# uzh-rpg/rpg_svo

Hardware: AMD Instinct MI355X
Metric: frames/sec sparse-align+pose-refine (VGA, 4 pyr lvls); ATE vs CPU ref (higher is better)
Workload: dtype value = default build: K1 f32 pixels/residuals/chi2/per-pixel products, f64 Jacobian rows/partials/reductions/projection/solve/pose; K4 f64 (reference-width build: roofline_f64_build.value)

## Files before the change

rpg_svo_amd/csrc/sparse_align.hip:

```cpp
#include <cstdlib>
#include <map>
#include <mutex>
#include <utility>

#include "sia_common.h"

using namespace svo_capi;
using namespace svo_dev;
using namespace svo_sia;

namespace {

#define MINW(BLOCK) ((BLOCK) >= 256 ? 4 : 3)

#ifdef SIA_PROFILE
#define SIA_T() ((long long)__builtin_readcyclecounter())
#define SIA_ACC(k, t0, t1) prof[k] += (t1) - (t0)
#else
#define SIA_T() 0ll
#define SIA_ACC(k, t0, t1)
#endif

constexpr int MAX_WAVES = SVO_HIP_MAX_PATCHES / 64;

#if defined(SIA_F64_PARTIALS)
using sia_pix = double;
using sia_acc = double;
#undef MINW
#define MINW(BLOCK) 3
#else
using sia_pix = float;
using sia_acc = double;
#endif

struct SplitModel {
  double q[2][4], t[2][3];
};

struct SiaLds {
  SplitModel sm;
  double Rt[12];
  int sw_done, sw_stop, sw_nmeas, sw_cur, sw_old;
  double sw_chi2;
  double H[21];
  double Hinv[36];
  double A[36];
  sia_acc part[2][MAX_WAVES][8];
  int chg[2][MAX_WAVES];
  int xfail;
  sia_acc Hpart[MAX_WAVES][24];
  long long lo[SVO_HIP_MAX_LEVELS];
  int lw[SVO_HIP_MAX_LEVELS];
  int lh[SVO_HIP_MAX_LEVELS];
  int lp[SVO_HIP_MAX_LEVELS];
};
__shared__ SiaLds g_s;


template <int PARTS>
__device__ __forceinline__ void sia_rebuild_hinv(int lane, int nw, [[maybe_unused]] XChunk* xh, [[maybe_unused]] int part,
                                                 [[maybe_unused]] unsigned gen, [[maybe_unused]] int& xfail) {
  asm volatile("" : "+v"(lane));
#ifndef SVO_HOST_MATH_TEST
  if constexpr (PARTS > 1) {
    static_assert((PARTS - 1) * 21 <= 64, "one lane per chunk of the other parts");
    const int j = lane / 21, k = lane - 21 * j;
    double v = 0.0;
    for (int w = 0; w < nw; ++w) v += (double)g_s.Hpart[w][k];
    if (j == 0) sia_xstore(xh + part * SIA_XH_SLOTS + k, v, gen);
    const int other = j < part ? j : j + 1;
    double got = 0.0;
    if (j < PARTS - 1) got = sia_xpoll(xh + other * SIA_XH_SLOTS + k, gen, xfail);
    if (xfail) g_s.xfail = 1;
    double tot = 0.0;
#pragma unroll
    for (int p = 0; p < PARTS; ++p) {
      const double theirs = __shfl(got, (p < part ? p : p - 1) * 21 + k, 64);
      const double term = p == part ? v : theirs;
      tot = p == 0 ? term : tot + term;
    }
    if (lane < 21) g_s.H[lane] = tot;
  } else
#endif
  if (lane < 21) {
    double v = 0.0;
    for (int w = 0; w < nw; ++w) v += (double)g_s.Hpart[w][lane];
    g_s.H[lane] = v;
  }
  SVO_WAVE_LDS_FENCE();
  const int gi = lane / 6, gj = lane - 6 * gi;
  if (lane < 36) {
    g_s.A[lane] = g_s.H[sym6_rt(gi, gj)];
    g_s.Hinv[lane] = (gi == gj) ? 1.0 : 0.0;
  }
  for (int k = 0; k < 6; ++k) {
    SVO_WAVE_LDS_FENCE();
    if (lane < 36) {
      const double p = g_s.A[k * 6 + k];
      const double aik = g_s.A[gi * 6 + k];
      const double akj = g_s.A[k * 6 + gj];
      const double bkj = g_s.Hinv[k * 6 + gj];
      const double aij = g_s.A[lane];
      const double bij = g_s.Hinv[lane];
      const double ip = (fabs(p) > 2.2250738585072014e-308) ? sia_rcp(p) : 0.0;
      const double na = (gi == k) ? akj * ip : aij - aik * (akj * ip);
      const double nb = (gi == k) ? bkj * ip : bij - aik * (bkj * ip);
      SVO_LANES_LDS_FENCE();
      g_s.A[lane] = na;
      g_s.Hinv[lane] = nb;
    }
  }
}


__device__ __forceinline__ float sia_bilerp(float wtl, float wtr, float wbl, float wbr, float tl, float tr, float bl, float br) {
  return __builtin_fmaf(wbr, br, __builtin_fmaf(wbl, bl, __builtin_fmaf(wtr, tr, wtl * tl)));
}
typedef float sia_f2 __attribute__((ext_vector_type(2)));
__device__ __forceinline__ sia_f2 sia_bilerp2(sia_f2 wtl, sia_f2 wtr, sia_f2 wbl, sia_f2 wbr, sia_f2 tl, sia_f2 tr, sia_f2 bl,
                                              sia_f2 br) {
  return __builtin_elementwise_fma(wbr, br, __builtin_elementwise_fma(wbl, bl, __builtin_elementwise_fma(wtr, tr, wtl * tl)));
}

#ifdef SIA_F64_PARTIALS
#define SIA_PACKED 0
#else
#define SIA_PACKED 1
#endif
template <int BLOCK, bool WC, bool DIST, int PARTS = 1>
__global__ void __launch_bounds__(BLOCK, PARTS > 1 ? 1 : ((DIST && BLOCK < 1024) ? 3 : MINW(BLOCK))) sia_kernel(const SiaArgs a) {
  constexpr int NW = BLOCK / 64;
  int b, part = 0;
  if constexpr (PARTS > 1) {
    b = (int)(blockIdx.x / (8 * PARTS)) * 8 + (int)(blockIdx.x % 8);
    part = (int)(blockIdx.x / 8) % PARTS;
    if (b >= a.B) return;
  } else {
    b = (int)xcd_contiguous_block();
  }
  [[maybe_unused]] XChunk* const xbase = PARTS > 1 ? static_cast<XChunk*>(a.xw) + (size_t)b * SIA_X_BLOCK : nullptr;
  [[maybe_unused]] unsigned xseq = 0;
#ifndef SVO_HOST_MATH_TEST
  if constexpr (PARTS > 1) xseq = (unsigned)__builtin_amdgcn_readfirstlane((int)sia_xload(xbase + SIA_X_CHUNKS).lo);
#endif
  [[maybe_unused]] int xfail = 0;
  const int tid = threadIdx.x;
  const int lane = tid & 63;
  const int wave = tid >> 6;

  __shared__ float4 s_bt[8][BLOCK];

  int n = a.n[b];
  n = n > a.n_stride ? a.n_stride : n;
  const svo_hip_sia_params P = a.P;

  if (n <= 0) {
    if (tid == 0 && part == 0) {
      for (int k = 0; k < 12; ++k) a.T_out[12 * b + k] = a.T_in[12 * b + k];
      if (a.H_out)
        for (int k = 0; k < 36; ++k) a.H_out[36 * b + k] = 0.0;
      a.n_tracked[b] = 0;
      if (a.iters)
        for (int k = 0; k < SVO_HIP_MAX_LEVELS; ++k) a.iters[SVO_HIP_MAX_LEVELS * b + k] = 0;
      if (a.chi2) a.chi2[b] = 1e10;
      if (a.status) a.status[b] = 0;
    }
    return;
  }

  const int pid = part * BLOCK + tid;
  const size_t fo = (size_t)b * a.n_stride + pid;
  const bool has = (pid < n) && (a.valid ? a.valid[fo] != 0 : true);
  double X = 0, Y = 0, Z = 1;
  if (has) {
    X = a.xyz[3 * fo];
    Y = a.xyz[3 * fo + 1];
    Z = a.xyz[3 * fo + 2];
  }
  double px_kept0 = 0, px_kept1 = 0;
  if (has) {
    px_kept0 = a.px[2 * fo];
    px_kept1 = a.px[2 * fo + 1];
  }
  const double rz = sia_rcp(Z);
  const sia_acc zi = (sia_acc)rz;
  const sia_acc xn = (sia_acc)(X * rz);
  const sia_acc yn = (sia_acc)(Y * rz);
  const uint8_t* ref_base = a.store + (int64_t)a.ref_slot[b] * a.L.slot_bytes;
  const uint8_t* cur_base = a.store + (int64_t)a.cur_slot[b] * a.L.slot_bytes;

  if (tid == 0) {
#pragma unroll
    for (int k = 0; k < SVO_HIP_MAX_LEVELS; ++k) {
      g_s.lw[k] = a.L.w[k];
      g_s.lh[k] = a.L.h[k];
      g_s.lp[k] = a.L.pitch[k];
      g_s.lo[k] = a.L.offset[k];
    }
    for (int k = 0; k < 21; ++k) g_s.H[k] = 0.0;
    g_s.xfail = 0;
    if (a.iters && part == 0)
      for (int k = 0; k < SVO_HIP_MAX_LEVELS; ++k) a.iters[SVO_HIP_MAX_LEVELS * b + k] = 0;
  }
  double R[9], tr[3];
  {
    double q[4];
    for (int k = 0; k < 9; ++k) R[k] = a.T_in[12 * b + k];
    for (int k = 0; k < 3; ++k) tr[k] = a.T_in[12 * b + 9 + k];
    quat_from_R(R, q);
    quat_to_R(q, R);
    if (tid == 0) {
      for (int k = 0; k < 4; ++k) g_s.sm.q[0][k] = q[k];
      for (int k = 0; k < 3; ++k) g_s.sm.t[0][k] = tr[k];
    }
  }
  int m_cur = 0, m_old = 0;
  double chi2_prev = 1e10;
  int stop = 0;
  int n_meas_last = 0;
  int buf = 0;

  const int sw = (NW > 1) ? (int)(blockIdx.x % NW) : 0;
  sia_pix Sxx = 0, Sxy = 0, Syy = 0;
  sia_acc gmask = 0;
  bool vis = false;

  __syncthreads();

#ifdef SIA_PROFILE
  long long prof[8] = {0, 0, 0, 0, 0, 0, 0, 0};
  const long long t_begin = SIA_T();
#endif
  for (int level = P.max_level; level >= P.min_level; --level) {
    [[maybe_unused]] const long long tl0 = SIA_T();
    const int cols = g_s.lw[level], rows = g_s.lh[level], pitch = g_s.lp[level];
    const uint8_t* ref_img = ref_base + g_s.lo[level];
    const uint8_t* cur_img = cur_base + g_s.lo[level];
    const float scale = pow2_inv_f32(level);
    const sia_acc fl = (sia_acc)(fabs(P.fx) * pow2_inv_f64(level));

    uint32_t wc[WC ? 7 : 1][3];
    int wc_u0 = 0, wc_v0 = -100000;
    if (WC) {
#pragma unroll
      for (int r = 0; r < (WC ? 7 : 1); ++r) wc[r][0] = wc[r][1] = wc[r][2] = 0u;
    }
    {
      const double pxx = px_kept0, pxy = px_kept1;
      const float u_ref = (float)(pxx * (double)scale);
      const float v_ref = (float)(pxy * (double)scale);
      const int u_i = (int)floorf(u_ref);
      const int v_i = (int)floorf(v_ref);
      const bool inb = has && !(u_i - 3 < 0 || v_i - 3 < 0 || u_i + 3 >= cols || v_i + 3 >= rows);
      Sxx = Sxy = Syy = 0;
      if (inb) {
        vis = true;
        gmask = 1;
        const float su = u_ref - (float)u_i, sv = v_ref - (float)v_i;
        const float wtl = (1.f - su) * (1.f - sv);
        const float wtr = su * (1.f - sv);
        const float wbl = (1.f - su) * sv;
        const float wbr = su * sv;
        float Bt[6][6];
        float Wp[7], Wc[7];
        uint32_t rw[7][3];
        const int rxa = run_start(u_i - 3, 7);
        const uint32_t rbo = (uint32_t)(u_i - 3 - rxa);
        load_window12<7>(ref_img, pitch, rxa, v_i - 3, rw);
        cut_row7(rw[0], rbo, Wp);
#pragma unroll
        for (int r = 0; r < 6; ++r) {
          cut_row7(rw[r + 1], rbo, Wc);
#pragma unroll
          for (int c = 0; c < 6; ++c) {
            const bool need = ((r >= 1 && r <= 4)) || ((c >= 1 && c <= 4));
            if (need) Bt[r][c] = sia_bilerp(wtl, wtr, wbl, wbr, Wp[c], Wp[c + 1], Wc[c], Wc[c + 1]);
          }
#pragma unroll
          for (int c = 0; c < 7; ++c) Wp[c] = Wc[c];
        }
#pragma unroll
        for (int y = 0; y < 4; ++y)
#pragma unroll
          for (int x = 0; x < 4; ++x) {
            const float dx = 0.5f * (Bt[y + 1][x + 2] - Bt[y + 1][x]);
            const float dy = 0.5f * (Bt[y + 2][x + 1] - Bt[y][x + 1]);
            Sxx += (sia_pix)dx * (sia_pix)dx;
            Sxy += (sia_pix)dx * (sia_pix)dy;
            Syy += (sia_pix)dy * (sia_pix)dy;
          }
#if SIA_PACKED
        s_bt[0][tid] = make_float4(Bt[0][1], Bt[0][3], Bt[0][2], Bt[0][4]);
        s_bt[1][tid] = make_float4(Bt[1][0], Bt[1][2], Bt[1][1], Bt[1][3]);
        s_bt[2][tid] = make_float4(Bt[1][4], Bt[1][5], Bt[2][0], Bt[2][2]);
        s_bt[3][tid] = make_float4(Bt[2][1], Bt[2][3], Bt[2][4], Bt[2][5]);
        s_bt[4][tid] = make_float4(Bt[3][0], Bt[3][2], Bt[3][1], Bt[3][3]);
        s_bt[5][tid] = make_float4(Bt[3][4], Bt[3][5], Bt[4][0], Bt[4][2]);
        s_bt[6][tid] = make_float4(Bt[4][1], Bt[4][3], Bt[4][4], Bt[4][5]);
        s_bt[7][tid] = make_float4(Bt[5][1], Bt[5][3], Bt[5][2], Bt[5][4]);
#else
        s_bt[0][tid] = make_float4(Bt[0][1], Bt[0][2], Bt[0][3], Bt[0][4]);
        s_bt[1][tid] = make_float4(Bt[1][0], Bt[1][1], Bt[1][2], Bt[1][3]);
        s_bt[2][tid] = make_float4(Bt[1][4], Bt[1][5], Bt[2][0], Bt[2][1]);
        s_bt[3][tid] = make_float4(Bt[2][2], Bt[2][3], Bt[2][4], Bt[2][5]);
        s_bt[4][tid] = make_float4(Bt[3][0], Bt[3][1], Bt[3][2], Bt[3][3]);
        s_bt[5][tid] = make_float4(Bt[3][4], Bt[3][5], Bt[4][0], Bt[4][1]);
        s_bt[6][tid] = make_float4(Bt[4][2], Bt[4][3], Bt[4][4], Bt[4][5]);
        s_bt[7][tid] = make_float4(Bt[5][1], Bt[5][2], Bt[5][3], Bt[5][4]);
#endif
      } else {
        gmask = 0;
      }
    }

    m_old = m_cur;
    int inH = -1;
    int evals = 0;
    SIA_ACC(5, tl0, SIA_T());
    for (int iter = 0; iter < P.n_iter; ++iter) {
      [[maybe_unused]] const long long tp0 = SIA_T();
      bool m = false;
      sia_pix gx = 0, gy = 0;
      float c2 = 0.f;
      if (vis) {
        const double xc = R[0] * X + R[1] * Y + R[2] * Z + tr[0];
        const double yc = R[3] * X + R[4] * Y + R[5] * Z + tr[1];
        const double zc = R[6] * X + R[7] * Y + R[8] * Z + tr[2];
        double izc = __builtin_amdgcn_rcp(zc);
        izc = fma(fma(-zc, izc, 1.0), izc, izc);
        izc = fma(fma(-zc, izc, 1.0), izc, izc);
        double pu, pv;
        if (DIST) {
          Cam cm;
          cm.fx = P.fx; cm.fy = P.fy; cm.cx = P.cx; cm.cy = P.cy;
          cm.width = 0; cm.height = 0;
          cm.model = P.cam_model;
#pragma unroll
          for (int k = 0; k < 5; ++k) cm.d[k] = P.d[k];
          const double uvn[2] = {xc * izc, yc * izc};
          double pxd[2];
          world2cam_uv(cm, uvn, pxd);
          pu = pxd[0];
          pv = pxd[1];
        } else {
          pu = P.fx * (xc * izc) + P.cx;
          pv = P.fy * (yc * izc) + P.cy;
        }
        const float u_cur = (float)pu * scale;
        const float v_cur = (float)pv * scale;
        const float fu = floorf(u_cur), fv = floorf(v_cur);
        if (fu - 3.f >= 0.f && fv - 3.f >= 0.f && fu + 3.f < (float)cols && fv + 3.f < (float)rows) {
          m = true;
          const int u_i = (int)fu, v_i = (int)fv;
          const float su = u_cur - fu, sv = v_cur - fv;
          const float wtl = (1.f - su) * (1.f - sv);
          const float wtr = su * (1.f - sv);
          const float wbl = (1.f - su) * sv;
          const float wbr = su * sv;
          {
#if SIA_PACKED
          typedef float f2 __attribute__((ext_vector_type(2)));
          uint32_t cw[5][3];
          uint32_t cbo = 0;
          uint64_t k0 = 0, k1 = 0, kup = 0;
          int bo = 0;
          if (WC) {
            int r0 = (v_i - 2) - wc_v0;
            bo = (u_i - 2) - wc_u0;
            if (!(r0 >= 0 && r0 <= 2 && bo >= 0 && bo <= 7)) {
              wc_v0 = v_i - 3;
              wc_u0 = run_start(u_i - 3, 7);
              load_window12<(WC ? 7 : 1)>(cur_img, pitch, wc_u0, wc_v0, wc);
              r0 = 1;
              bo = (u_i - 2) - wc_u0;
            }
            k0 = SVO_BALLOT_ACTIVE(r0 == 0);
            k1 = SVO_BALLOT_ACTIVE(r0 == 1);
            kup = SVO_BALLOT_ACTIVE(bo >= 4);
          } else {
            const int cxa = run_start(u_i - 2, 5);
            cbo = (uint32_t)(u_i - 2 - cxa);
            load_window12<5>(cur_img, pitch, cxa, v_i - 2, cw);
          }
#define SIA_WIN_ROW(r, p02, p13, p24)                                                                                   \
  do {                                                                                                                  \
    float o_[5];                                                                                                        \
    if (WC) {                                                                                                           \
      constexpr int S_ = WC ? 1 : 0;                                                                                    \
      const uint32_t d0_ = sel_e64(k0, wc[(r) * S_][0], sel_e64(k1, wc[((r) + 1) * S_][0], wc[((r) + 2) * S_][0]));     \
      const uint32_t d1_ = sel_e64(k0, wc[(r) * S_][1], sel_e64(k1, wc[((r) + 1) * S_][1], wc[((r) + 2) * S_][1]));     \
      const uint32_t d2_ = sel_e64(k0, wc[(r) * S_][2], sel_e64(k1, wc[((r) + 1) * S_][2], wc[((r) + 2) * S_][2]));     \
      cut_row5(d0_, d1_, d2_, bo, kup, o_);                                                                             \
    } else {                                                                                                            \
      cut_row5_plain(cw[WC ? 0 : (r)], cbo, o_);                                                                        \
    }                                                                                                                   \
    p02 = f2{o_[0], o_[2]};                                                                                             \
    p13 = f2{o_[1], o_[3]};                                                                                             \
    p24 = f2{o_[2], o_[4]};                                                                                             \
  } while (0)
          const float2* const bt2 = reinterpret_cast<const float2*>(&s_bt[0][0]);
#define SIA_BT2(q, h) bt2[((q) * BLOCK + tid) * 2 + (h)]
          const f2 vtl = f2{wtl, wtl}, vtr = f2{wtr, wtr}, vbl = f2{wbl, wbl}, vbr = f2{wbr, wbr};
          f2 c2v = f2{0.f, 0.f}, gxv = f2{0.f, 0.f}, gyv = f2{0.f, 0.f};
          f2 t02, t13, t24, b02, b13, b24;
          SIA_WIN_ROW(0, t02, t13, t24);
          SIA_WIN_ROW(1, b02, b13, b24);
          f2 a13, a24, b02t, b13t, b45t, c02, c13, c45;
          { const float2 v0 = SIA_BT2(0, 0), v1 = SIA_BT2(0, 1); a13 = f2{v0.x, v0.y}; a24 = f2{v1.x, v1.y}; }
          { const float2 v0 = SIA_BT2(1, 0), v1 = SIA_BT2(1, 1), v2 = SIA_BT2(2, 0);
            b02t = f2{v0.x, v0.y}; b13t = f2{v1.x, v1.y}; b45t = f2{v2.x, v2.y}; }
          { const float2 v0 = SIA_BT2(2, 1), v1 = SIA_BT2(3, 0), v2 = SIA_BT2(3, 1);
            c02 = f2{v0.x, v0.y}; c13 = f2{v1.x, v1.y}; c45 = f2{v2.x, v2.y}; }
#pragma unroll
          for (int y = 0; y < 4; ++y) {
            f2 n02 = f2{0.f, 0.f}, n13 = f2{0.f, 0.f}, n45 = f2{0.f, 0.f};
            if (y == 0) { const float2 v0 = SIA_BT2(4, 0), v1 = SIA_BT2(4, 1), v2 = SIA_BT2(5, 0);
                          n02 = f2{v0.x, v0.y}; n13 = f2{v1.x, v1.y}; n45 = f2{v2.x, v2.y}; }
            if (y == 1) { const float2 v0 = SIA_BT2(5, 1), v1 = SIA_BT2(6, 0), v2 = SIA_BT2(6, 1);
                          n02 = f2{v0.x, v0.y}; n13 = f2{v1.x, v1.y}; n45 = f2{v2.x, v2.y}; }
            if (y == 2) { const float2 v0 = SIA_BT2(7, 0), v1 = SIA_BT2(7, 1);
                          n13 = f2{v0.x, v0.y}; n45 = f2{v1.x, v1.y}; }
            const f2 b24t = f2{b02t.y, b45t.x}, b35t = f2{b13t.y, b45t.y};
            const f2 c24 = (y < 3) ? f2{c02.y, c45.x} : c45;
            const f2 Ia = sia_bilerp2(vtl, vtr, vbl, vbr, t02, t13, b02, b13);
            const f2 Ib = sia_bilerp2(vtl, vtr, vbl, vbr, t13, t24, b13, b24);
            const f2 ra = Ia - b13t, rb = Ib - b24t;
            c2v += ra * ra;
            c2v += rb * rb;
            gxv += ra * (b24t - b02t);
            gxv += rb * (b35t - b13t);
            gyv += ra * (c13 - a13);
            gyv += rb * (c24 - a24);
            if (y < 3) {
              f2 w02, w13, w24;
              SIA_WIN_ROW(y + 2, w02, w13, w24);
              t02 = b02; t13 = b13; t24 = b24;
              b02 = w02; b13 = w13; b24 = w24;
              a13 = b13t; a24 = b24t;
              b02t = c02; b13t = c13; b45t = c45;
              c02 = n02; c13 = n13; c45 = n45;
              asm volatile("" ::: "memory");
            }
          }
#undef SIA_WIN_ROW
#undef SIA_BT2
          c2 += c2v.x + c2v.y;
          gx += gxv.x + gxv.y;
          gy += gyv.x + gyv.y;
#else
          float W[5][5];
          if (WC) {
            int r0 = (v_i - 2) - wc_v0;
            int bo = (u_i - 2) - wc_u0;
            if (!(r0 >= 0 && r0 <= 2 && bo >= 0 && bo <= 7)) {
              wc_v0 = v_i - 3;
              wc_u0 = run_start(u_i - 3, 7);
              load_window12<(WC ? 7 : 1)>(cur_img, pitch, wc_u0, wc_v0, wc);
              r0 = 1;
              bo = (u_i - 2) - wc_u0;
            }
            const uint64_t k0 = SVO_BALLOT_ACTIVE(r0 == 0), k1 = SVO_BALLOT_ACTIVE(r0 == 1);
            const uint64_t kup = SVO_BALLOT_ACTIVE(bo >= 4);
#pragma unroll
            for (int r = 0; r < 5; ++r) {
              constexpr int S = WC ? 1 : 0;
              const uint32_t d0 = sel_e64(k0, wc[r * S][0], sel_e64(k1, wc[(r + 1) * S][0], wc[(r + 2) * S][0]));
              const uint32_t d1 = sel_e64(k0, wc[r * S][1], sel_e64(k1, wc[(r + 1) * S][1], wc[(r + 2) * S][1]));
              const uint32_t d2 = sel_e64(k0, wc[r * S][2], sel_e64(k1, wc[(r + 1) * S][2], wc[(r + 2) * S][2]));
              cut_row5(d0, d1, d2, bo, kup, W[r]);
            }
          } else {
            uint32_t cw[5][3];
            const int cxa = run_start(u_i - 2, 5);
            const uint32_t cbo = (uint32_t)(u_i - 2 - cxa);
            load_window12<5>(cur_img, pitch, cxa, v_i - 2, cw);
#pragma unroll
            for (int r = 0; r < 5; ++r) cut_row5_plain(cw[r], cbo, W[r]);
          }
          float Bt[6][6];
          {
            const float4 q0 = s_bt[0][tid], q1 = s_bt[1][tid], q2 = s_bt[2][tid], q3 = s_bt[3][tid];
            const float4 q4 = s_bt[4][tid], q5 = s_bt[5][tid], q6 = s_bt[6][tid], q7 = s_bt[7][tid];
            Bt[0][0] = Bt[0][5] = Bt[5][0] = Bt[5][5] = 0.f;
            Bt[0][1] = q0.x; Bt[0][2] = q0.y; Bt[0][3] = q0.z; Bt[0][4] = q0.w;
            Bt[1][0] = q1.x; Bt[1][1] = q1.y; Bt[1][2] = q1.z; Bt[1][3] = q1.w;
            Bt[1][4] = q2.x; Bt[1][5] = q2.y; Bt[2][0] = q2.z; Bt[2][1] = q2.w;
            Bt[2][2] = q3.x; Bt[2][3] = q3.y; Bt[2][4] = q3.z; Bt[2][5] = q3.w;
            Bt[3][0] = q4.x; Bt[3][1] = q4.y; Bt[3][2] = q4.z; Bt[3][3] = q4.w;
            Bt[3][4] = q5.x; Bt[3][5] = q5.y; Bt[4][0] = q5.z; Bt[4][1] = q5.w;
            Bt[4][2] = q6.x; Bt[4][3] = q6.y; Bt[4][4] = q6.z; Bt[4][5] = q6.w;
            Bt[5][1] = q7.x; Bt[5][2] = q7.y; Bt[5][3] = q7.z; Bt[5][4] = q7.w;
          }
#pragma unroll
          for (int y = 0; y < 4; ++y)
#pragma unroll
            for (int x = 0; x < 4; ++x) {
              const float I = sia_bilerp(wtl, wtr, wbl, wbr, W[y][x], W[y][x + 1], W[y + 1][x], W[y + 1][x + 1]);
              const float res = I - Bt[y + 1][x + 1];
              c2 += res * res;
              gx += (sia_pix)res * (sia_pix)(Bt[y + 1][x + 2] - Bt[y + 1][x]);
              gy += (sia_pix)res * (sia_pix)(Bt[y + 2][x + 1] - Bt[y][x + 1]);
            }
#endif
          }
        }
      }
      {
        const sia_acc gsc = (sia_acc)0.5 * fl * gmask;
        const sia_acc gxf = m ? (sia_acc)gx * gsc : (sia_acc)0, gyf = m ? (sia_acc)gy * gsc : (sia_acc)0;
        sia_acc part[8];
        sia_acc zi_ = zi, xn_ = xn, yn_ = yn;
        asm volatile("" : "+v"(zi_), "+v"(xn_), "+v"(yn_));
        part[0] = zi_ * gxf;
        part[1] = zi_ * gyf;
        part[2] = -zi_ * (xn_ * gxf + yn_ * gyf);
        part[3] = -(xn_ * yn_ * gxf + ((sia_acc)1 + yn_ * yn_) * gyf);
        part[4] = ((sia_acc)1 + xn_ * xn_) * gxf + xn_ * yn_ * gyf;
        part[5] = xn_ * gyf - yn_ * gxf;
        part[6] = (sia_acc)c2;
        part[7] = m ? (sia_acc)16 : (sia_acc)0;
        [[maybe_unused]] const long long tp1 = SIA_T();
        SIA_ACC(0, tp0, tp1);
        const sia_acc tot = wave_reduce8(part, lane);
        if ((lane & 7) == 0) g_s.part[buf][wave][lane >> 3] = tot;
        const int mine = __builtin_amdgcn_ballot_w64((int)m != inH) != 0ull;
        if (lane == 0) g_s.chg[buf][wave] = mine;
        SIA_ACC(1, tp1, SIA_T());
      }
      [[maybe_unused]] const long long tb0 = SIA_T();
      __syncthreads();
      int changed = 0;
#pragma unroll
      for (int w = 0; w < NW; ++w) changed |= g_s.chg[buf][w];
      [[maybe_unused]] double xtot = 0.0;
#ifndef SVO_HOST_MATH_TEST
      if constexpr (PARTS > 1) {
        ++xseq;
        const int xp = lane >> 4, xk = lane & 15;
        double own = 0.0;
        if (xk < 8) {
#pragma unroll
          for (int w = 0; w < NW; ++w) own += (double)g_s.part[buf][w][xk];
        } else if (xk == 8) {
          own = (double)changed;
        }
        XChunk* const slot = xbase + (size_t)(xseq & 1) * (SIA_X_MAX_PARTS * SIA_X_SLOTS);
        if (wave == sw && xp == part && xk < 9) sia_xstore(slot + part * SIA_X_SLOTS + xk, own, xseq);
        double val = own;
        if (xp != part && xp < PARTS && xk < 9) val = sia_xpoll(slot + xp * SIA_X_SLOTS + xk, xseq, xfail);
        if (xfail) g_s.xfail = 1;
        xtot = __shfl(val, xk, 64);
#pragma unroll
        for (int p = 1; p < PARTS; ++p) xtot += __shfl(val, 16 * p + xk, 64);
        changed = readlane_f64<8>(xtot) != 0.0;
      }
#endif
      [[maybe_unused]] const long long tb1 = SIA_T();
      SIA_ACC(2, tb0, tb1);
      if (changed) {
        sia_acc zi_ = zi, xn_ = xn, yn_ = yn;
        asm volatile("" : "+v"(zi_), "+v"(xn_), "+v"(yn_));
        const sia_acc one = 1, zero = 0;
        const sia_acc ja[6] = {-zi_ * fl, zero, xn_ * zi_ * fl, xn_ * yn_ * fl, -(one + xn_ * xn_) * fl, yn_ * fl};
        const sia_acc jb[6] = {zero, -zi_ * fl, yn_ * zi_ * fl, (one + yn_ * yn_) * fl, -xn_ * yn_ * fl, -xn_ * fl};
        sia_acc hp[24];
#pragma unroll
        for (int i = 0; i < 6; ++i)
#pragma unroll
          for (int j = i; j < 6; ++j) {
            const sia_acc v = (sia_acc)Sxx * (ja[i] * ja[j]) + (sia_acc)Sxy * (ja[i] * jb[j] + jb[i] * ja[j]) + (sia_acc)Syy * (jb[i] * jb[j]);
            hp[sym6(i, j)] = m ? v : zero;
          }
        hp[21] = hp[22] = hp[23] = zero;
#pragma unroll
        for (int g = 0; g < 3; ++g) {
          const sia_acc tot = wave_reduce8(hp + 8 * g, lane);
          if ((lane & 7) == 0) g_s.Hpart[wave][8 * g + (lane >> 3)] = tot;
        }
        inH = (int)m;
        __syncthreads();
        if constexpr (PARTS > 1) {
          ++xseq;
          XChunk* const xh = xbase + 2 * SIA_X_MAX_PARTS * SIA_X_SLOTS + (size_t)(xseq & 1) * (SIA_X_MAX_PARTS * SIA_XH_SLOTS);
          if (wave == 0) sia_rebuild_hinv<PARTS>(lane, NW, xh, part, xseq, xfail);
        } else {
          if (wave == 0) sia_rebuild_hinv<1>(lane, NW, nullptr, 0, 0u, xfail);
        }
        __syncthreads();
      }
      ++evals;
      [[maybe_unused]] const long long ts0 = SIA_T();
      SIA_ACC(3, tb1, ts0);
#ifdef SIA_PROFILE
      prof[7] += 1;
#endif

      int done = 0;
      const int swb = (NW > 1) ? (sw + 1) % NW : sw;
      const bool rot_wave = wave == sw, trans_wave = wave == swb;
      int m_next = m_cur;
      if (rot_wave || trans_wave) {
        __builtin_amdgcn_s_setprio(3);
        double colsum = 0.0;
        if constexpr (PARTS > 1) {
          colsum = xtot;
        } else {
          const int k = lane & 7;
#pragma unroll
          for (int w = 0; w < NW; ++w) colsum += (double)g_s.part[buf][w][k];
        }
        const double b0 = readlane_f64<0>(colsum), b1 = readlane_f64<1>(colsum), b2 = readlane_f64<2>(colsum);
        const double b3 = readlane_f64<3>(colsum), b4 = readlane_f64<4>(colsum), b5 = readlane_f64<5>(colsum);
        const float chi2_sum = (float)readlane_f64<6>(colsum);
        const int n_meas = (int)readlane_f64<7>(colsum);
        double xi;
        {
          const double* row = &g_s.Hinv[6 * (lane < 6 ? lane : 0)];
          xi = row[0] * b0 + row[1] * b1 + row[2] * b2 + row[3] * b3 + row[4] * b4 + row[5] * b5;
        }
        const double x0 = readlane_f64<0>(xi), x1 = readlane_f64<1>(xi), x2 = readlane_f64<2>(xi);
        const double x3 = readlane_f64<3>(xi), x4 = readlane_f64<4>(xi), x5 = readlane_f64<5>(xi);
        n_meas_last = n_meas;
        const double new_chi2 = (double)(chi2_sum / (float)n_meas);
        if (isnan(x0)) stop = 1;
        const SplitModel& sm = g_s.sm;
        const bool rollback = (iter > 0 && new_chi2 > chi2_prev) || stop;
        if (rollback) {
          m_next = m_old;
          done = 1;
        } else {
          m_next = m_cur ^ 1;
          m_old = m_cur;
          chi2_prev = new_chi2;
          const double nm = fmax(fmax(fmax(fabs(x0), fabs(x1)), fmax(fabs(x2), fabs(x3))), fmax(fabs(x4), fabs(x5)));
          if (nm <= P.eps) done = 1;
        }
        const float mx[6] = {-(float)x0, -(float)x1, -(float)x2, -(float)x3, -(float)x4, -(float)x5};
        if (rot_wave) {
          double q[4];
          if (rollback) {
#pragma unroll
            for (int k = 0; k < 4; ++k) q[k] = sm.q[m_next][k];
          } else {
#ifdef SIA_F64_PARTIALS
            const double mxd[6] = {-x0, -x1, -x2, -x3, -x4, -x5};
            double eq[4], et_unused[3];
            se3_exp(mxd, eq, et_unused);
#else
            float eqf[4];
            se3_exp_rot_f32(mx, eqf);
            const double eq[4] = {eqf[0], eqf[1], eqf[2], eqf[3]};
#endif
            double oq[4];
#pragma unroll
            for (int k = 0; k < 4; ++k) oq[k] = sm.q[m_cur][k];
            quat_mul(oq, eq, q);
            quat_normalize_fast(q);
            if (lane == 0) {
#pragma unroll
              for (int k = 0; k < 4; ++k) g_s.sm.q[m_next][k] = q[k];
            }
          }
          quat_to_R(q, R);
          if (lane == 0) {
#pragma unroll
            for (int k = 0; k < 9; ++k) g_s.Rt[k] = R[k];
            g_s.sw_done = done;
            g_s.sw_stop = stop;
            g_s.sw_nmeas = n_meas_last;
            g_s.sw_chi2 = chi2_prev;
            g_s.sw_cur = m_next;
            g_s.sw_old = m_old;
          }
        }
        if (trans_wave) {
          if (rollback) {
#pragma unroll
            for (int k = 0; k < 3; ++k) tr[k] = sm.t[m_next][k];
          } else {
#ifdef SIA_F64_PARTIALS
            const double mxd[6] = {-x0, -x1, -x2, -x3, -x4, -x5};
            double eq_unused[4], et[3];
            se3_exp(mxd, eq_unused, et);
#else
            float etf[3];
            se3_exp_trans_f32(mx, etf);
            const double et[3] = {etf[0], etf[1], etf[2]};
#endif
            double oq[4], rt[3];
#pragma unroll
            for (int k = 0; k < 4; ++k) oq[k] = sm.q[m_cur][k];
            quat_rot(oq, et, rt);
#pragma unroll
            for (int k = 0; k < 3; ++k) tr[k] = sm.t[m_cur][k] + rt[k];
            if (lane == 0) {
#pragma unroll
              for (int k = 0; k < 3; ++k) g_s.sm.t[m_next][k] = tr[k];
            }
          }
          if (lane == 0) {
#pragma unroll
            for (int k = 0; k < 3; ++k) g_s.Rt[9 + k] = tr[k];
          }
        }
        __builtin_amdgcn_s_setprio(0);
      }
      m_cur = m_next;
      if (NW > 1) {
        __syncthreads();
#pragma unroll
        for (int k = 0; k < 9; ++k) R[k] = g_s.Rt[k];
#pragma unroll
        for (int k = 0; k < 3; ++k) tr[k] = g_s.Rt[9 + k];
        done = g_s.sw_done;
        stop = g_s.sw_stop;
        n_meas_last = g_s.sw_nmeas;
        chi2_prev = g_s.sw_chi2;
        m_cur = g_s.sw_cur;
        m_old = g_s.sw_old;
      }
      buf ^= 1;
      SIA_ACC(4, ts0, SIA_T());
      if (done) break;
    }
    if (tid == 0 && part == 0 && a.iters) a.iters[SVO_HIP_MAX_LEVELS * b + level] = evals;
  }

  if (tid == 0 && part == 0) {
    for (int k = 0; k < 9; ++k) a.T_out[12 * b + k] = R[k];
    for (int k = 0; k < 3; ++k) a.T_out[12 * b + 9 + k] = tr[k];
    if (a.H_out)
      for (int i = 0; i < 6; ++i)
        for (int j = 0; j < 6; ++j) a.H_out[36 * b + i * 6 + j] = g_s.H[sym6_rt(i, j)];
#ifdef SIA_PROFILE
    prof[6] = SIA_T() - t_begin;
    if (a.H_out)
      for (int k = 0; k < 8; ++k) a.H_out[36 * b + k] = (double)prof[k];
#endif
    a.n_tracked[b] = n_meas_last / 16;
    if (a.chi2) a.chi2[b] = chi2_prev;
    if constexpr (PARTS > 1) {
#ifndef SVO_HOST_MATH_TEST
      sia_xstore_epoch(xbase + SIA_X_CHUNKS, xseq + (g_s.xfail ? (1u << 16) : 0u));
#endif
    }
    if (a.status) a.status[b] = (stop ? SVO_HIP_SIA_STOP : 0) | ((PARTS > 1 && g_s.xfail) ? SVO_HIP_SIA_EXCHANGE_TIMEOUT : 0);
  }
}


template <int BLOCK>
int launch(const SiaArgs& args, int B, hipStream_t s) {
  constexpr bool WC = BLOCK == 256;
  if (args.P.cam_model == SVO_HIP_CAM_PINHOLE)
    hipLaunchKernelGGL((sia_kernel<BLOCK, WC, false>), dim3(B), dim3(BLOCK), 0, s, args);
  else
    hipLaunchKernelGGL((sia_kernel<BLOCK, false, true>), dim3(B), dim3(BLOCK), 0, s, args);
  return check_launch();
}

}

namespace {

int sia_prepare(const svo_hip_pyr_layout* layout, const uint8_t* d_store, int B, const int32_t* d_ref_slot,
                const int32_t* d_cur_slot, const int32_t* d_n, int n_stride, const double* d_px, const double* d_xyz_ref,
                const uint8_t* d_valid, const svo_hip_sia_params* params, const double* d_T_in, double* d_T_out,
                double* d_H_out, int32_t* d_n_tracked, int32_t* d_iters, double* d_chi2, int32_t* d_status, SiaArgs* out) {
  if (!layout_ok(layout) || !d_store || !params || B < 0) return SVO_HIP_EINVAL;
  if (B == 0) return SVO_HIP_OK;
  if (!d_ref_slot || !d_cur_slot || !d_n || !d_px || !d_xyz_ref || !d_T_in || !d_T_out || !d_n_tracked)
    return SVO_HIP_EINVAL;
  if (n_stride < 1) return SVO_HIP_EINVAL;
  if (n_stride > SVO_HIP_MAX_PATCHES) return SVO_HIP_ERANGE;
  if (params->min_level < 0 || params->max_level < params->min_level || params->max_level >= layout->n_levels ||
      params->n_iter < 0)
    return SVO_HIP_EINVAL;
  if (params->cam_model != SVO_HIP_CAM_PINHOLE && params->cam_model != SVO_HIP_CAM_PINHOLE_RADTAN &&
      params->cam_model != SVO_HIP_CAM_ATAN)
    return SVO_HIP_EINVAL;
  SiaArgs& args = *out;
  args.L = *layout;
  args.store = d_store;
  args.ref_slot = d_ref_slot;
  args.cur_slot = d_cur_slot;
  args.n = d_n;
  args.n_stride = n_stride;
  args.px = d_px;
  args.xyz = d_xyz_ref;
  args.valid = d_valid;
  args.P = *params;
  args.T_in = d_T_in;
  args.T_out = d_T_out;
  args.H_out = d_H_out;
  args.n_tracked = d_n_tracked;
  args.iters = d_iters;
  args.chi2 = d_chi2;
  args.status = d_status;
  return 1;
}

constexpr int SIA_SPLIT_PARTS = 4;
constexpr int SIA_SPLIT_MAX_B = 128;
#ifndef SVO_HOST_MATH_TEST
bool sia_split_applies(const SiaArgs& args, int B) {
  static const bool on = [] { const char* v = std::getenv("SVO_HIP_K1_SPLIT"); return !(v && v[0] == '0'); }();
  return on && args.n_stride > 512 && B <= SIA_SPLIT_MAX_B;
}
void* sia_split_blocks(hipStream_t s) {
  static std::mutex mut;
  static std::map<std::pair<int, hipStream_t>, void*> blocks;
  int dev = 0;
  if (hipGetDevice(&dev) != hipSuccess) return nullptr;
  std::lock_guard<std::mutex> g(mut);
  void*& p = blocks[std::make_pair(dev, s)];
  if (p) return p;
  hipStreamCaptureStatus cap = hipStreamCaptureStatusNone;
  if (hipStreamIsCapturing(s, &cap) != hipSuccess || cap != hipStreamCaptureStatusNone) return nullptr;
  const size_t bytes = (size_t)SIA_SPLIT_MAX_B * SIA_X_BLOCK * sizeof(XChunk);
  void* q = nullptr;
  if (hipMalloc(&q, bytes) != hipSuccess) return nullptr;
  if (hipMemset(q, 0, bytes) != hipSuccess || hipDeviceSynchronize() != hipSuccess) {
    (void)hipFree(q);
    return nullptr;
  }
  p = q;
  return p;
}
int launch_split(SiaArgs args, int B, void* xw, hipStream_t s) {
  args.B = B;
  args.xw = xw;
  const dim3 grid((unsigned)((B + 7) / 8) * 8 * SIA_SPLIT_PARTS), blk(256);
  if (args.P.cam_model == SVO_HIP_CAM_PINHOLE)
    hipLaunchKernelGGL((sia_kernel<256, true, false, SIA_SPLIT_PARTS>), grid, blk, 0, s, args);
  else
    hipLaunchKernelGGL((sia_kernel<256, false, true, SIA_SPLIT_PARTS>), grid, blk, 0, s, args);
  return check_launch();
}
#endif

int launch_workgroup(const SiaArgs& args, int B, hipStream_t s) {
  if (args.n_stride <= 64) return launch<64>(args, B, s);
  if (args.n_stride <= 128) return launch<128>(args, B, s);
  if (args.n_stride <= 256) return launch<256>(args, B, s);
  if (args.n_stride <= 512) return launch<512>(args, B, s);
  return launch<1024>(args, B, s);
}

}

extern "C" int svo_hip_sparse_align(const svo_hip_pyr_layout* layout, const uint8_t* d_store, int B,
                                    const int32_t* d_ref_slot, const int32_t* d_cur_slot, const int32_t* d_n,
                                    int n_stride, const double* d_px, const double* d_xyz_ref,
                                    const uint8_t* d_valid, const svo_hip_sia_params* params,
                                    const double* d_T_in, double* d_T_out, double* d_H_out,
                                    int32_t* d_n_tracked, int32_t* d_iters, double* d_chi2, int32_t* d_status,
                                    void* stream) {
  SiaArgs args;
  const int rc = sia_prepare(layout, d_store, B, d_ref_slot, d_cur_slot, d_n, n_stride, d_px, d_xyz_ref, d_valid, params,
                             d_T_in, d_T_out, d_H_out, d_n_tracked, d_iters, d_chi2, d_status, &args);
  if (rc <= 0) return rc;
  hipStream_t s = static_cast<hipStream_t>(stream);
  if (sia_wave_applies(args, B)) return launch_sia_wave(args, B, s);
#ifndef SVO_HOST_MATH_TEST
  if (sia_split_applies(args, B))
    if (void* xw = sia_split_blocks(s)) return launch_split(args, B, xw, s);
#endif
  return launch_workgroup(args, B, s);
}

extern "C" int svo_hip_sparse_align_workgroup(const svo_hip_pyr_layout* layout, const uint8_t* d_store, int B,
                                              const int32_t* d_ref_slot, const int32_t* d_cur_slot, const int32_t* d_n,
                                              int n_stride, const double* d_px, const double* d_xyz_ref,
                                              const uint8_t* d_valid, const svo_hip_sia_params* params,
                                              const double* d_T_in, double* d_T_out, double* d_H_out,
                                              int32_t* d_n_tracked, int32_t* d_iters, double* d_chi2,
                                              int32_t* d_status, void* stream) {
  SiaArgs args;
  const int rc = sia_prepare(layout, d_store, B, d_ref_slot, d_cur_slot, d_n, n_stride, d_px, d_xyz_ref, d_valid, params,
                             d_T_in, d_T_out, d_H_out, d_n_tracked, d_iters, d_chi2, d_status, &args);
  if (rc <= 0) return rc;
  return launch_workgroup(args, B, static_cast<hipStream_t>(stream));
}
```

Measured before the change: 11.50 million.

## Fold Hessian rebuild into solver waves and drop extra block barriers

In the single-part path, each wave now recomputes and reduces its Hessian partial only when its own mask changed, and does so before the existing barrier. The separate barrier-bracketed Hinv rebuild by wave 0 is removed. Instead the rotation and translation solver waves each sum the partials and invert H redundantly into their own double-buffered Hinv/A slots. This removes two __syncthreads per changed iteration. In exchange, two waves repeat the 6x6 inversion and the LDS footprint of Hinv and A grows.

Result: no change. 11.47 million, median of 3 (-0.3%).

```diff
diff --git a/rpg_svo_amd/csrc/sparse_align.hip b/rpg_svo_amd/csrc/sparse_align.hip
--- a/rpg_svo_amd/csrc/sparse_align.hip
+++ b/rpg_svo_amd/csrc/sparse_align.hip
@@ -43,8 +43,8 @@
   int sw_done, sw_stop, sw_nmeas, sw_cur, sw_old;
   double sw_chi2;
   double H[21];
-  double Hinv[36];
-  double A[36];
+  double Hinv[2][36];
+  double A[2][36];
   sia_acc part[2][MAX_WAVES][8];
   int chg[2][MAX_WAVES];
   int xfail;
@@ -89,27 +89,88 @@
   }
   SVO_WAVE_LDS_FENCE();
   const int gi = lane / 6, gj = lane - 6 * gi;
+  double* const A = g_s.A[0];
+  double* const Hinv = g_s.Hinv[0];
   if (lane < 36) {
-    g_s.A[lane] = g_s.H[sym6_rt(gi, gj)];
-    g_s.Hinv[lane] = (gi == gj) ? 1.0 : 0.0;
+    A[lane] = g_s.H[sym6_rt(gi, gj)];
+    Hinv[lane] = (gi == gj) ? 1.0 : 0.0;
   }
   for (int k = 0; k < 6; ++k) {
     SVO_WAVE_LDS_FENCE();
     if (lane < 36) {
-      const double p = g_s.A[k * 6 + k];
-      const double aik = g_s.A[gi * 6 + k];
-      const double akj = g_s.A[k * 6 + gj];
-      const double bkj = g_s.Hinv[k * 6 + gj];
-      const double aij = g_s.A[lane];
-      const double bij = g_s.Hinv[lane];
+      const double p = A[k * 6 + k];
+      const double aik = A[gi * 6 + k];
+      const double akj = A[k * 6 + gj];
+      const double bkj = Hinv[k * 6 + gj];
+      const double aij = A[lane];
+      const double bij = Hinv[lane];
       const double ip = (fabs(p) > 2.2250738585072014e-308) ? sia_rcp(p) : 0.0;
       const double na = (gi == k) ? akj * ip : aij - aik * (akj * ip);
       const double nb = (gi == k) ? bkj * ip : bij - aik * (bkj * ip);
       SVO_LANES_LDS_FENCE();
-      g_s.A[lane] = na;
-      g_s.Hinv[lane] = nb;
-    }
-  }
+      A[lane] = na;
+      Hinv[lane] = nb;
+    }
+  }
+}
+
+template <typename PIX>
+__device__ __forceinline__ void sia_h_partial(PIX Sxx, PIX Sxy, PIX Syy, sia_acc zi, sia_acc xn, sia_acc yn, sia_acc fl, bool m,
+                                              int lane, int wave) {
+  sia_acc zi_ = zi, xn_ = xn, yn_ = yn;
+  asm volatile("" : "+v"(zi_), "+v"(xn_), "+v"(yn_));
+  const sia_acc one = 1, zero = 0;
+  const sia_acc ja[6] = {-zi_ * fl, zero, xn_ * zi_ * fl, xn_ * yn_ * fl, -(one + xn_ * xn_) * fl, yn_ * fl};
+  const sia_acc jb[6] = {zero, -zi_ * fl, yn_ * zi_ * fl, (one + yn_ * yn_) * fl, -xn_ * yn_ * fl, -xn_ * fl};
+  sia_acc hp[24];
+#pragma unroll
+  for (int i = 0; i < 6; ++i)
+#pragma unroll
+    for (int j = i; j < 6; ++j) {
+      const sia_acc v = (sia_acc)Sxx * (ja[i] * ja[j]) + (sia_acc)Sxy * (ja[i] * jb[j] + jb[i] * ja[j]) + (sia_acc)Syy * (jb[i] * jb[j]);
+      hp[sym6(i, j)] = m ? v : zero;
+    }
+  hp[21] = hp[22] = hp[23] = zero;
+#pragma unroll
+  for (int g = 0; g < 3; ++g) {
+    const sia_acc tot = wave_reduce8(hp + 8 * g, lane);
+    if ((lane & 7) == 0) g_s.Hpart[wave][8 * g + (lane >> 3)] = tot;
+  }
+}
+
+template <int NW>
+__device__ __forceinline__ void sia_solver_hinv(int lane, bool write_h, double* Hinv, double* A) {
+  asm volatile("" : "+v"(lane));
+  double s = 0.0;
+  if (lane < 21) {
+#pragma unroll
+    for (int w = 0; w < NW; ++w) s += (double)g_s.Hpart[w][lane];
+    if (write_h) g_s.H[lane] = s;
+  }
+  const int gi = lane / 6, gj = lane - 6 * gi;
+  const double h = __shfl(s, sym6_rt(gi, gj), 64);
+  if (lane < 36) {
+    A[lane] = h;
+    Hinv[lane] = (gi == gj) ? 1.0 : 0.0;
+  }
+  for (int k = 0; k < 6; ++k) {
+    SVO_WAVE_LDS_FENCE();
+    if (lane < 36) {
+      const double p = A[k * 6 + k];
+      const double aik = A[gi * 6 + k];
+      const double akj = A[k * 6 + gj];
+      const double bkj = Hinv[k * 6 + gj];
+      const double aij = A[lane];
+      const double bij = Hinv[lane];
+      const double ip = (fabs(p) > 2.2250738585072014e-308) ? sia_rcp(p) : 0.0;
+      const double na = (gi == k) ? akj * ip : aij - aik * (akj * ip);
+      const double nb = (gi == k) ? bkj * ip : bij - aik * (bkj * ip);
+      SVO_LANES_LDS_FENCE();
+      A[lane] = na;
+      Hinv[lane] = nb;
+    }
+  }
+  SVO_WAVE_LDS_FENCE();
 }
 
 
@@ -229,6 +290,7 @@
 
 #ifdef SIA_PROFILE
   long long prof[8] = {0, 0, 0, 0, 0, 0, 0, 0};
+  long long prof_rebuilds = 0;
   const long long t_begin = SIA_T();
 #endif
   for (int level = P.max_level; level >= P.min_level; --level) {
@@ -526,6 +588,14 @@
         const int mine = __builtin_amdgcn_ballot_w64((int)m != inH) != 0ull;
         if (lane == 0) g_s.chg[buf][wave] = mine;
         SIA_ACC(1, tp1, SIA_T());
+        if constexpr (PARTS == 1) {
+          if (mine) {
+            [[maybe_unused]] const long long th0 = SIA_T();
+            sia_h_partial(Sxx, Sxy, Syy, zi, xn, yn, fl, m, lane, wave);
+            inH = (int)m;
+            SIA_ACC(3, th0, SIA_T());
+          }
+        }
       }
       [[maybe_unused]] const long long tb0 = SIA_T();
       __syncthreads();
@@ -557,37 +627,20 @@
 #endif
       [[maybe_unused]] const long long tb1 = SIA_T();
       SIA_ACC(2, tb0, tb1);
-      if (changed) {
-        sia_acc zi_ = zi, xn_ = xn, yn_ = yn;
-        asm volatile("" : "+v"(zi_), "+v"(xn_), "+v"(yn_));
-        const sia_acc one = 1, zero = 0;
-        const sia_acc ja[6] = {-zi_ * fl, zero, xn_ * zi_ * fl, xn_ * yn_ * fl, -(one + xn_ * xn_) * fl, yn_ * fl};
-        const sia_acc jb[6] = {zero, -zi_ * fl, yn_ * zi_ * fl, (one + yn_ * yn_) * fl, -xn_ * yn_ * fl, -xn_ * fl};
-        sia_acc hp[24];
-#pragma unroll
-        for (int i = 0; i < 6; ++i)
-#pragma unroll
-          for (int j = i; j < 6; ++j) {
-            const sia_acc v = (sia_acc)Sxx * (ja[i] * ja[j]) + (sia_acc)Sxy * (ja[i] * jb[j] + jb[i] * ja[j]) + (sia_acc)Syy * (jb[i] * jb[j]);
-            hp[sym6(i, j)] = m ? v : zero;
-          }
-        hp[21] = hp[22] = hp[23] = zero;
-#pragma unroll
-        for (int g = 0; g < 3; ++g) {
-          const sia_acc tot = wave_reduce8(hp + 8 * g, lane);
-          if ((lane & 7) == 0) g_s.Hpart[wave][8 * g + (lane >> 3)] = tot;
-        }
-        inH = (int)m;
-        __syncthreads();
-        if constexpr (PARTS > 1) {
+      if constexpr (PARTS > 1) {
+        if (changed) {
+          sia_h_partial(Sxx, Sxy, Syy, zi, xn, yn, fl, m, lane, wave);
+          inH = (int)m;
+          __syncthreads();
           ++xseq;
           XChunk* const xh = xbase + 2 * SIA_X_MAX_PARTS * SIA_X_SLOTS + (size_t)(xseq & 1) * (SIA_X_MAX_PARTS * SIA_XH_SLOTS);
           if (wave == 0) sia_rebuild_hinv<PARTS>(lane, NW, xh, part, xseq, xfail);
-        } else {
-          if (wave == 0) sia_rebuild_hinv<1>(lane, NW, nullptr, 0, 0u, xfail);
-        }
-        __syncthreads();
+          __syncthreads();
+        }
       }
+#ifdef SIA_PROFILE
+      prof_rebuilds += changed ? 1 : 0;
+#endif
       ++evals;
       [[maybe_unused]] const long long ts0 = SIA_T();
       SIA_ACC(3, tb1, ts0);
@@ -601,6 +654,11 @@
       int m_next = m_cur;
       if (rot_wave || trans_wave) {
         __builtin_amdgcn_s_setprio(3);
+        const int hslot = (PARTS == 1 && !rot_wave) ? 1 : 0;
+        double* const hinv = g_s.Hinv[hslot];
+        if constexpr (PARTS == 1) {
+          if (changed) sia_solver_hinv<NW>(lane, rot_wave, hinv, g_s.A[hslot]);
+        }
         double colsum = 0.0;
         if constexpr (PARTS > 1) {
           colsum = xtot;
@@ -615,7 +673,7 @@
         const int n_meas = (int)readlane_f64<7>(colsum);
         double xi;
         {
-          const double* row = &g_s.Hinv[6 * (lane < 6 ? lane : 0)];
+          const double* row = &hinv[6 * (lane < 6 ? lane : 0)];
           xi = row[0] * b0 + row[1] * b1 + row[2] * b2 + row[3] * b3 + row[4] * b4 + row[5] * b5;
         }
         const double x0 = readlane_f64<0>(xi), x1 = readlane_f64<1>(xi), x2 = readlane_f64<2>(xi);
@@ -736,6 +794,7 @@
     prof[6] = SIA_T() - t_begin;
     if (a.H_out)
       for (int k = 0; k < 8; ++k) a.H_out[36 * b + k] = (double)prof[k];
+    if (a.H_out) a.H_out[36 * b + 8] = (double)prof_rebuilds;
 #endif
     a.n_tracked[b] = n_meas_last / 16;
     if (a.chi2) a.chi2[b] = chi2_prev;
```
